# SamsungLabs/fcaf3d

Hardware: AMD Instinct MI355X
Metric: scenes/sec fwd+bwd, ScanNet 100k-pt 2cm voxels, 1/2/4/8 MI355X (higher is better)
Workload: dtype f32

## Files before the change

fcaf3d_amd/_lib.py:

```python
import ctypes
import os
import re
import threading
import time

import torch

_HERE = os.path.dirname(os.path.abspath(__file__))
LIB_PATH = os.environ.get('FC_LIB') or os.path.join(_HERE, 'libfcaf3d_hip.so')
HEADER = os.path.join(os.path.dirname(_HERE), 'include', 'fcaf3d_hip.h')

_SCALARS = {'int': ctypes.c_int, 'int64_t': ctypes.c_int64, 'float': ctypes.c_float,
            'hipStream_t': ctypes.c_void_p}


def parse_header(path=HEADER):
    txt = open(path).read()
    txt = re.sub(r'/\*.*?\*/', '', txt, flags=re.S)
    protos = {}
    for m in re.finditer(r'\b(int64_t|int)\s+(fc_\w+)\s*\(([^)]*)\)\s*;', txt):
        ret, name, args = m.group(1), m.group(2), m.group(3)
        argl = []
        for a in args.split(','):
            a = ' '.join(a.split())
# ... 15 lines not shown
    txt = re.sub(r'//[^\n]*', '', open(path).read())
    known, blocks = {}, []
    for m in re.finditer(r'\benum\s*\{([^}]*)\}', txt):
        block, nxt = {}, 0
        for item in filter(None, (s.strip() for s in m.group(1).split(','))):
            name, _, expr = (s.strip() for s in item.partition('='))
            if expr:
                nxt = sum(known[t] if t in known else int(t, 0) for t in (s.strip() for s in expr.split('+')))
            assert re.fullmatch(r'[A-Z]\w*', name) and name not in known, item
            block[name] = known[name] = nxt
            nxt += 1
        blocks.append(block)
    return blocks


ABI_VERSION = 14
_lib = None
_protos = None


def lib():
    global _lib, _protos
    if _lib is None:
        if not os.path.exists(LIB_PATH):
            raise RuntimeError(
                f'{LIB_PATH} is missing: build it with `python -m fcaf3d_amd.build` '
                '(hipcc --offload-arch=gfx950).  There is no CPU fallback.')
        l = ctypes.CDLL(LIB_PATH)
        _protos = parse_header()
        for name, (ret, args) in _protos.items():
            fn = getattr(l, name)
# ... 119 lines not shown
```

fcaf3d_amd/csrc/exec.hip:

```cpp
#include "fc_common.h"
#include "../../include/fcaf3d_hip.h"
#include "exec_ops.h"
#include <vector>

namespace {

constexpr int MAX_EVENTS = 64;

constexpr int MAX_DEVICES = 16;
hipEvent_t g_events_dev[MAX_DEVICES][MAX_EVENTS];
bool g_events_ready[MAX_DEVICES] = {};
thread_local hipEvent_t* g_events = nullptr;

int ensure_events() {
  int dev = 0;
  FC_HIP(hipGetDevice(&dev));
  if (dev < 0 || dev >= MAX_DEVICES) return FC_EINVAL;
  if (!g_events_ready[dev]) {
    for (int i = 0; i < MAX_EVENTS; ++i) FC_HIP(hipEventCreateWithFlags(&g_events_dev[dev][i], hipEventDisableTiming));
    g_events_ready[dev] = true;
  }
  g_events = g_events_dev[dev];
  return 0;
}
// ... 382 lines not shown
    }
    case OP_AMAX: {
      if (c.dry) return 0;
      return fc_amax(P<const float>(c, op[AMAX_X]), c.dims[op[AMAX_N]] * op[AMAX_C], P<unsigned>(c, op[AMAX_SLOT]), st);
    }
    case OP_CLEAR: {
      if (c.dry) return 0;
      FC_HIP(hipMemsetAsync(P<void>(c, op[CLEAR_DST]), 0, (size_t)op[CLEAR_BYTES], st));
      return 0;
    }
    case OP_NORM_POOL_FWD: {
      const int64_t* m = c.maps + op[NORM_POOL_FWD_MAP] * MAPW;
      if (c.dry) return 0;
      if ((int)m[MAP_K] != 8) return FC_EINVAL;
      if (op[NORM_POOL_FWD_AMAX_OUT_P1] > 0) fc_amax_out_hint(P1<unsigned>(c, op[NORM_POOL_FWD_AMAX_OUT_P1]));
      return fc_norm_act_maxpool8_fwd(P<const float>(c, op[NORM_POOL_FWD_X]), P<const int>(c, op[NORM_POOL_FWD_SEG]),
                                      op[NORM_POOL_FWD_SEG] >= 0 ? 4 : 0, (int)op[NORM_POOL_FWD_C], P<const float>(c, op[NORM_POOL_FWD_MEAN]),
                                      P<const float>(c, op[NORM_POOL_FWD_VAR]), (float)as_double(op[NORM_POOL_FWD_EPS]),
                                      P<const float>(c, op[NORM_POOL_FWD_GAMMA]), P<const float>(c, op[NORM_POOL_FWD_BETA]),
                                      (int)op[NORM_POOL_FWD_ACT], reinterpret_cast<const int*>(m[MAP_NBR]), m[MAP_N_OUT],
                                      P<float>(c, op[NORM_POOL_FWD_OUT]), P<int>(c, op[NORM_POOL_FWD_ARG]), P<float>(c, op[NORM_POOL_FWD_Y]),
                                      P<int>(c, op[NORM_POOL_FWD_PARENT]), st);
    }
    case OP_POOL_NORM_BWD: {
      const int64_t n = c.dims[op[POOL_NORM_BWD_N]];
      const int C = (int)op[POOL_NORM_BWD_C], nseg = (int)c.dims[op[POOL_NORM_BWD_NSEG]];
      if (!want_ws(c, s, fc_maxpool8_norm_act_bwd_ws_bytes(n, C, nseg))) return 0;
      return fc_maxpool8_norm_act_bwd(P<const float>(c, op[POOL_NORM_BWD_X]), P<const float>(c, op[POOL_NORM_BWD_G_POOL]),
                                      P<const int>(c, op[POOL_NORM_BWD_ARG]), P<const int>(c, op[POOL_NORM_BWD_PARENT]),
                                      P<const int>(c, op[POOL_NORM_BWD_SEG]), op[POOL_NORM_BWD_SEG] >= 0 ? 4 : 0, n, C, nseg,
                                      P<const float>(c, op[POOL_NORM_BWD_MEAN]), P<const float>(c, op[POOL_NORM_BWD_VAR]),
                                      P<const float>(c, op[POOL_NORM_BWD_CNT]), (float)as_double(op[POOL_NORM_BWD_EPS]),
                                      P<const float>(c, op[POOL_NORM_BWD_GAMMA]), P<const float>(c, op[POOL_NORM_BWD_BETA]),
                                      (int)op[POOL_NORM_BWD_ACT], P<float>(c, op[POOL_NORM_BWD_GX]), P<float>(c, op[POOL_NORM_BWD_SUMS]),
                                      c.ws[s], c.ws_bytes[s], st);
    }
    case OP_INV_ROWS: {
      if (c.dry) return 0;
      return fc_inverse_rows(P<const int>(c, op[INV_ROWS_ROWS]), c.dims[op[INV_ROWS_N]], c.dims[op[INV_ROWS_N_INV]], P<int>(c, op[INV_ROWS_INV]), st);
    }
    case OP_COPY: {
      if (c.dry) return 0;
// ... 72 lines not shown
```

fcaf3d_amd/csrc/exec_ops.h:

```cpp
#ifndef FCAF3D_EXEC_OPS_H
#define FCAF3D_EXEC_OPS_H

enum {
  OPW = 24,
  MAPW = 20,
  NSTREAM = 3
};
enum { ROW_OP, ROW_STREAM };

enum {
  OP_STEM_FWD = 1, OP_COL_STATS, OP_NORM_FWD, OP_MAXPOOL_FWD, OP_CONV, OP_BN_FWD, OP_UNION_FWD, OP_HEAD_FWD, OP_RECORD, OP_WAIT,
  OP_HEAD_BWD, OP_WGRAD, OP_BN_BWD, OP_NORM_BWD, OP_MAXPOOL_BWD, OP_STEM_WGRAD, OP_GATHER, OP_ADD, OP_SMALL_GRADS,
  OP_PERMUTE_GENT, OP_HEAD_WFIN, OP_COPY, OP_COL_SUM, OP_ROW_SUM, OP_AMAX, OP_CLEAR, OP_NORM_POOL_FWD, OP_POOL_NORM_BWD, OP_INV_ROWS
};

enum {
  STEM_FWD_X = 2,
  STEM_FWD_W,
  STEM_FWD_MAP,
  STEM_FWD_OUT,
  STEM_FWD_COL,
  STEM_FWD_END
};
enum {
// ... 206 lines not shown
  NORM_POOL_FWD_X = 2,
  NORM_POOL_FWD_SEG,
  NORM_POOL_FWD_C,
  NORM_POOL_FWD_MEAN,
  NORM_POOL_FWD_VAR,
  NORM_POOL_FWD_EPS,
  NORM_POOL_FWD_GAMMA,
  NORM_POOL_FWD_BETA,
  NORM_POOL_FWD_ACT,
  NORM_POOL_FWD_MAP,
  NORM_POOL_FWD_OUT,
  NORM_POOL_FWD_ARG,
  NORM_POOL_FWD_Y,
  NORM_POOL_FWD_AMAX_OUT_P1,
  NORM_POOL_FWD_PARENT,
  NORM_POOL_FWD_END
};
enum {
  POOL_NORM_BWD_X = 2,
  POOL_NORM_BWD_G_POOL,
  POOL_NORM_BWD_ARG,
  POOL_NORM_BWD_PARENT,
  POOL_NORM_BWD_SEG,
  POOL_NORM_BWD_N,
  POOL_NORM_BWD_C,
  POOL_NORM_BWD_NSEG,
  POOL_NORM_BWD_MEAN,
  POOL_NORM_BWD_VAR,
  POOL_NORM_BWD_CNT,
  POOL_NORM_BWD_EPS,
  POOL_NORM_BWD_GAMMA,
  POOL_NORM_BWD_BETA,
  POOL_NORM_BWD_ACT,
  POOL_NORM_BWD_GX,
  POOL_NORM_BWD_SUMS,
  POOL_NORM_BWD_END
};
enum {
  INV_ROWS_ROWS = 2,
  INV_ROWS_N,
  INV_ROWS_N_INV,
  INV_ROWS_INV,
  INV_ROWS_END
};

static_assert(STEM_FWD_END <= OPW && COL_STATS_END <= OPW && CONV_END <= OPW && BN_FWD_END <= OPW && HEAD_FWD_END <= OPW, "operator row");
static_assert(RECORD_END <= OPW && WAIT_END <= OPW && HEAD_BWD_END <= OPW && WGRAD_END <= OPW && BN_BWD_END <= OPW, "operator row");
static_assert(STEM_WGRAD_END <= OPW && GATHER_END <= OPW && ADD_END <= OPW && SMALL_GRADS_END <= OPW && PERMUTE_GENT_END <= OPW, "operator row");
static_assert(HEAD_WFIN_END <= OPW && COPY_END <= OPW && COL_SUM_END <= OPW && ROW_SUM_END <= OPW && AMAX_END <= OPW, "operator row");
static_assert(CLEAR_END <= OPW && NORM_POOL_FWD_END <= OPW && POOL_NORM_BWD_END <= OPW && INV_ROWS_END <= OPW, "operator row");
// ... 33 lines not shown
```

fcaf3d_amd/csrc/norm.hip:

```cpp
#include "fc_common.h"
#include "../../include/fcaf3d_hip.h"
#include "norm_route.h"

__device__ static inline int seg_of(const int* seg, int seg_stride, int64_t row) {
  return seg ? seg[row * seg_stride] : 0;
}

__device__ static inline void seg_range(const int* seg, int seg_stride, int64_t r0, int64_t r1, int* lo, int* hi,
                                        int* sh ) {
  if (!seg) { *lo = 0; *hi = 0; return; }
  if (threadIdx.x == 0) { sh[0] = 0x7fffffff; sh[1] = -1; }
  __syncthreads();
  int l = 0x7fffffff, h = -1;
  for (int64_t r = r0 + threadIdx.x; r < r1; r += blockDim.x) {
    int s = seg[r * seg_stride];
    l = s < l ? s : l;
    h = s > h ? s : h;
  }
  if (h >= 0) { atomicMin(&sh[0], l); atomicMax(&sh[1], h); }
  __syncthreads();
  *lo = sh[0]; *hi = sh[1];
  __syncthreads();
}

// ... 210 lines not shown
  if (residual) {
    float4 rs = *reinterpret_cast<const float4*>(residual + r * C + c);
    o.x += rs.x; o.y += rs.y; o.z += rs.z; o.w += rs.w;
  }
  o.x = act_fwd(o.x, act); o.y = act_fwd(o.y, act); o.z = act_fwd(o.z, act); o.w = act_fwd(o.w, act);
  if (q >= 0) {
    const float4 f = *reinterpret_cast<const float4*>(add_src + (int64_t)q * C + c);
    o.x += f.x; o.y += f.y; o.z += f.z; o.w += f.w;
  }
  *reinterpret_cast<float4*>(y + r * C + c) = o;
  amax_fold(am, o.x); amax_fold(am, o.y); amax_fold(am, o.z); amax_fold(am, o.w);
  }
  if (amax_out) amax_commit(am, amax_out);
}

template <bool POOL>
__global__ void k_norm_bwd_partial(const float* __restrict__ x, const float* __restrict__ y, const float* __restrict__ gy,
                                   const float* __restrict__ gy2, const int* __restrict__ pool_parent,
                                   const int* __restrict__ pool_arg, const int* __restrict__ seg, int seg_stride, int64_t n, int C, int nseg,
                                   const float* __restrict__ mean, const float* __restrict__ var, float eps, int act,
                                   const float* __restrict__ gamma, const float* __restrict__ beta,
                                   int64_t rpb, float* __restrict__ part) {
  extern __shared__ float sm[];
  __shared__ int srange[2];
  const int c4n = C / 4;
  const int cl = threadIdx.x % c4n, rl = threadIdx.x / c4n;
  const int nrl = blockDim.x / c4n;
  const int64_t r0 = (int64_t)blockIdx.x * rpb;
  int64_t r1 = r0 + rpb;
  if (r1 > n) r1 = n;
  int s_lo, s_hi;
// ... 9 lines not shown
      float4 is = make_float4(1.f / sqrtf(va.x + eps), 1.f / sqrtf(va.y + eps), 1.f / sqrtf(va.z + eps),
                              1.f / sqrtf(va.w + eps));
      const float4 gm = gamma ? *reinterpret_cast<const float4*>(gamma + cl * 4) : make_float4(1.f, 1.f, 1.f, 1.f);
      const float4 bt = beta ? *reinterpret_cast<const float4*>(beta + cl * 4) : make_float4(0.f, 0.f, 0.f, 0.f);
      const bool from_y = act && y;
      for (int64_t rb = r0 + rl; rb < r1; rb += 4 * nrl) {
        float4 xv[4], gv[4], yv[4], g2[4];
        bool ok[4];
#pragma unroll
        for (int u = 0; u < 4; ++u) {
          const int64_t r = rb + (int64_t)u * nrl;
          ok[u] = r < r1;
          const int64_t rc = ok[u] ? r : r0;
          if (chk) ok[u] = ok[u] && seg[rc * seg_stride] == s;
          xv[u] = *reinterpret_cast<const float4*>(x + rc * C + cl * 4);
          if (POOL) {
            const int64_t o = pool_parent[rc];
            const int4 a = *reinterpret_cast<const int4*>(pool_arg + o * C + cl * 4);
            gv[u] = *reinterpret_cast<const float4*>(gy + o * C + cl * 4);
            gv[u].x = a.x == rc ? gv[u].x : 0.f; gv[u].y = a.y == rc ? gv[u].y : 0.f;
            gv[u].z = a.z == rc ? gv[u].z : 0.f; gv[u].w = a.w == rc ? gv[u].w : 0.f;
          } else {
            gv[u] = *reinterpret_cast<const float4*>(gy + rc * C + cl * 4);
          }
          if (gy2) g2[u] = *reinterpret_cast<const float4*>(gy2 + rc * C + cl * 4);
          if (from_y) yv[u] = *reinterpret_cast<const float4*>(y + rc * C + cl * 4);
        }
#pragma unroll
        for (int u = 0; u < 4; ++u) {
          if (!ok[u]) continue;
          float4 g = gv[u];
// ... 24 lines not shown
    if (rl == 0) {
      float4 t1 = make_float4(0.f, 0.f, 0.f, 0.f), t2 = t1;
      for (int j = 0; j < nrl; ++j) {
        float4 u = *reinterpret_cast<const float4*>(&sm[(j * 2 + 0) * C + cl * 4]);
        float4 w = *reinterpret_cast<const float4*>(&sm[(j * 2 + 1) * C + cl * 4]);
        t1.x += u.x; t1.y += u.y; t1.z += u.z; t1.w += u.w;
        t2.x += w.x; t2.y += w.y; t2.z += w.z; t2.w += w.w;
      }
      float* dst = part + (((int64_t)blockIdx.x * nseg + s) * 2) * C;
      *reinterpret_cast<float4*>(dst + cl * 4) = t1;
      *reinterpret_cast<float4*>(dst + C + cl * 4) = t2;
    }
  }
}

template <bool POOL>
__global__ void k_norm_bwd_apply(const float* __restrict__ x, const float* __restrict__ y, const float* __restrict__ gy,
                                 const float* __restrict__ gy2, const int* __restrict__ pool_parent,
                                 const int* __restrict__ pool_arg, const int* __restrict__ seg, int seg_stride, int64_t n, int C,
                                 const float* __restrict__ mean, const float* __restrict__ var, float eps,
                                 const float* __restrict__ gamma, const float* __restrict__ beta,
                                 const float* __restrict__ sums ,
                                 const float* __restrict__ cnt, int act, float* __restrict__ gx, float* __restrict__ gres,
                                 unsigned* __restrict__ amax_out) {
  int64_t t = (int64_t)blockIdx.x * blockDim.x + threadIdx.x;
  const int c4n = C / 4;
  unsigned am = 0u;
  if (t < n * c4n) {
  int64_t r = t / c4n;
  int c = (int)(t % c4n) * 4;
  int s = seg_of(seg, seg_stride, r);
  float inv_n = 1.f / cnt[s];
  float xv[4], gv[4], muv[4], vav[4], gam[4], bet[4] = {0.f, 0.f, 0.f, 0.f}, s1[4], s2[4], yv[4], o[4], gr[4];
  *reinterpret_cast<float4*>(xv) = *reinterpret_cast<const float4*>(x + r * C + c);
  if (POOL) {
    const int64_t o = pool_parent[r];
    const int4 a = *reinterpret_cast<const int4*>(pool_arg + o * C + c);
    *reinterpret_cast<float4*>(gv) = *reinterpret_cast<const float4*>(gy + o * C + c);
    gv[0] = a.x == r ? gv[0] : 0.f; gv[1] = a.y == r ? gv[1] : 0.f; gv[2] = a.z == r ? gv[2] : 0.f; gv[3] = a.w == r ? gv[3] : 0.f;
  } else {
    *reinterpret_cast<float4*>(gv) = *reinterpret_cast<const float4*>(gy + r * C + c);
  }
  if (gy2) {
    const float4 t2 = *reinterpret_cast<const float4*>(gy2 + r * C + c);
    gv[0] += t2.x; gv[1] += t2.y; gv[2] += t2.z; gv[3] += t2.w;
  }
  *reinterpret_cast<float4*>(muv) = *reinterpret_cast<const float4*>(mean + (int64_t)s * C + c);
  *reinterpret_cast<float4*>(vav) = *reinterpret_cast<const float4*>(var + (int64_t)s * C + c);
  *reinterpret_cast<float4*>(s1) = *reinterpret_cast<const float4*>(sums + ((int64_t)s * 2) * C + c);
  *reinterpret_cast<float4*>(s2) = *reinterpret_cast<const float4*>(sums + ((int64_t)s * 2 + 1) * C + c);
// ... 69 lines not shown
  *reinterpret_cast<float4*>(out + o * C + c) = ob;
  *reinterpret_cast<int4*>(argrow + o * C + c) = make_int4(arg[0], arg[1], arg[2], arg[3]);
  amax_fold(am, ob.x); amax_fold(am, ob.y); amax_fold(am, ob.z); amax_fold(am, ob.w);
  }
  if (amax_out) amax_commit(am, amax_out);
}

__global__ void k_maxpool_bwd(const float* __restrict__ gout, const int* __restrict__ argrow, int64_t n_out, int C,
                              float* __restrict__ gin) {
  int64_t t = (int64_t)blockIdx.x * blockDim.x + threadIdx.x;
  if (t >= n_out * C) return;
  int i = argrow[t];
  if (i >= 0) gin[(int64_t)i * C + (t % C)] = gout[t];
}

__global__ void k_norm_act_maxpool8_fwd(const float* __restrict__ x, const int* __restrict__ seg, int seg_stride, int C,
                                        const float* __restrict__ mean, const float* __restrict__ var, float eps,
                                        const float* __restrict__ gamma, const float* __restrict__ beta, int act,
                                        const int* __restrict__ nbr, int64_t n_out, float* __restrict__ out, int* __restrict__ argrow,
                                        float* __restrict__ y, int* __restrict__ parent, unsigned* __restrict__ amax_out) {
  const int c4n = C / 4;
  int64_t t = (int64_t)blockIdx.x * blockDim.x + threadIdx.x;
  unsigned am = 0u;
  if (t < n_out * c4n) {
  const int64_t o = t / c4n;
  const int c = (int)(t % c4n) * 4;
  int idx[8];
#pragma unroll
  for (int k = 0; k < 8; ++k) idx[k] = nbr[(int64_t)k * n_out + o];
  if (parent) {
    int mine = -1;
#pragma unroll
    for (int k = 0; k < 8; ++k) mine = (c == 4 * k) ? idx[k] : mine;
    if (mine >= 0) parent[mine] = (int)o;
  }
  float4 v[8];
  int first = -1;
#pragma unroll
  for (int k = 0; k < 8; ++k) {
    const int i = idx[k] < 0 ? 0 : idx[k];
    if (first < 0 && idx[k] >= 0) first = idx[k];
    v[k] = *reinterpret_cast<const float4*>(x + (int64_t)i * C + c);
  }
  float best[4] = {-INFINITY, -INFINITY, -INFINITY, -INFINITY};
  int arg[4] = {-1, -1, -1, -1};
  if (first >= 0) {
    const int s = seg_of(seg, seg_stride, first);
    float mu[4], va[4], is[4], g[4] = {1.f, 1.f, 1.f, 1.f}, b[4] = {0.f, 0.f, 0.f, 0.f};
    *reinterpret_cast<float4*>(mu) = *reinterpret_cast<const float4*>(mean + (int64_t)s * C + c);
// ... 4 lines not shown
    for (int j = 0; j < 4; ++j) is[j] = 1.f / sqrtf(va[j] + eps);
#pragma unroll
    for (int k = 0; k < 8; ++k) {
      if (idx[k] < 0) continue;
      float e[4] = {v[k].x, v[k].y, v[k].z, v[k].w};
#pragma unroll
      for (int j = 0; j < 4; ++j) {
        e[j] = act_fwd(bn_pre(e[j], mu[j], is[j], g[j], b[j]), act);
        if (arg[j] < 0 || e[j] > best[j]) { best[j] = e[j]; arg[j] = idx[k]; }
      }
      if (y) *reinterpret_cast<float4*>(y + (int64_t)idx[k] * C + c) = make_float4(e[0], e[1], e[2], e[3]);
    }
  }
  float4 ob = make_float4(arg[0] < 0 ? 0.f : best[0], arg[1] < 0 ? 0.f : best[1], arg[2] < 0 ? 0.f : best[2], arg[3] < 0 ? 0.f : best[3]);
  *reinterpret_cast<float4*>(out + o * C + c) = ob;
  *reinterpret_cast<int4*>(argrow + o * C + c) = make_int4(arg[0], arg[1], arg[2], arg[3]);
  amax_fold(am, ob.x); amax_fold(am, ob.y); amax_fold(am, ob.z); amax_fold(am, ob.w);
  }
  if (amax_out) amax_commit(am, amax_out);
}

__global__ void k_inverse_rows(const int* __restrict__ rows, int64_t n, int64_t n_inv, int* __restrict__ inv) {
  const int64_t i = (int64_t)blockIdx.x * blockDim.x + threadIdx.x;
  if (i >= n) return;
  const int r = rows[i];
  if (r >= 0 && r < n_inv) inv[r] = (int)i;
}

__global__ void k_gather_rows(const float* __restrict__ src, const int* __restrict__ idx, int64_t n, int C,
                              float* __restrict__ dst) {
  int64_t t = (int64_t)blockIdx.x * blockDim.x + threadIdx.x;
// ... 456 lines not shown
    FC_CHECK_LAUNCH();
  }
  if (!apply) return FC_OK;
  if (r.apply == FC_NAPPLY_BN1)
    k_bn1_apply<<<FC_GRID(r.ap, stream)>>>(x, n, C, r.rpb, part, (int)r.np, eps, gamma, beta, residual, act, momentum, y, mean, var, cnt, rmean, rvar, nbt, add_inv, add_src);
  else if (r.apply == FC_NAPPLY_BN2)
    k_bn2_apply<<<FC_GRID(r.ap, stream)>>>(x, n, C, r.rpb, table, (int)r.np, groups, eps, gamma, beta, residual, act, momentum, y, mean, var, cnt, rmean, rvar, nbt, r.cg,
                                   add_inv, add_src, amax);
  else
    k_norm_act_fwd<<<FC_GRID(r.ap, stream)>>>(x, nullptr, 0, n, C, mean, var, eps, gamma, beta, residual, act, add_inv, add_src, y, amax);
  FC_CHECK_LAUNCH();
  if (r.amax == FC_NAMAX_PASS && amax) return fc_amax(y, n * (int64_t)C, amax, stream);
  return FC_OK;
}

template <bool POOL>
static int norm_bwd(int form, const float* x, const float* y, const float* gy, const float* gy2, const int* parent, const int* argrow, const int* seg,
                    int seg_stride, int64_t n, int C, int nseg, const float* mean, const float* var, const float* cnt, float eps, const float* gamma,
                    const float* beta, int act, float* gx, float* gres, float* sums, const float* table, int64_t nb_part, int64_t small_elems, void* ws,
                    int64_t ws_bytes, hipStream_t stream, unsigned* amax, bool late_hint = false) {
  if (act < 0 || act > 2) return FC_EINVAL;
  const NormRoute r = norm_bwd_route(n, C, nseg, table != nullptr, nb_part, small_elems, form);
  if (int rc = route_check(r, ws_bytes)) return rc;
  if (late_hint) amax = take_amax_out();
  if (r.apply == FC_NBAPPLY_NONE) {
    FC_HIP(hipMemsetAsync(sums, 0, sizeof(float) * nseg * 2 * C, stream));
    return FC_OK;
  }
  if (r.sums == FC_NRED_PARTIAL) {
    k_norm_bwd_partial<POOL><<<FC_GRID(r.red, stream)>>>(x, y, gy, gy2, parent, argrow, seg, seg_stride, n, C, nseg, mean, var, eps, act, gamma, beta, r.red_rpb, (float*)ws);
    FC_CHECK_LAUNCH();
// ... 93 lines not shown
  return bn_fwd(x, n, C, 0.f, nullptr, nullptr, nullptr, 0, momentum, nullptr, mean, var, cnt, running_mean, running_var, num_batches_tracked, nullptr, 0, 1,
                -1, nullptr, nullptr, ws, ws_bytes, stream, nullptr, false);
}

int fc_bn_act_train_fwd(const float* x, int64_t n, int C, float eps, const float* gamma, const float* beta,
                        const float* residual, int act, float momentum, float* y, float* mean, float* var, float* cnt,
                        float* running_mean, float* running_var, long long* num_batches_tracked, void* ws,
                        int64_t ws_bytes, hipStream_t stream) {
  return bn_fwd(x, n, C, eps, gamma, beta, residual, act, momentum, y, mean, var, cnt, running_mean, running_var, num_batches_tracked, nullptr, 0, 1,
                INT64_MAX, nullptr, nullptr, ws, ws_bytes, stream, nullptr);
}

int fc_bn_act_train_bwd(const float* x, const float* y, const float* gy, int64_t n, int C, const float* mean,
                        const float* var, float eps, const float* gamma, const float* beta, int act, float* gx, float* gres,
                        float* sums, void* ws, int64_t ws_bytes, hipStream_t stream) {
  return norm_bwd<false>(FC_NFORM_SMALL, x, y, gy, nullptr, nullptr, nullptr, nullptr, 0, n, C, 1, mean, var, nullptr, eps, gamma, beta, act, gx, gres, sums,
                         nullptr, 0, 0, ws, ws_bytes, stream, nullptr, true);
}

int fc_norm_act_add_fwd(const float* x, const int* seg, int seg_stride, int64_t n, int C, const float* mean, const float* var,
                        float eps, const float* gamma, const float* beta, const float* residual, int act, const int* add_inv,
                        const float* add_src, float* y, hipStream_t stream) {
  unsigned* ao = take_amax_out();
  if (n < 0 || C < 4 || C % 4 || act < 0 || act > 2 || (add_inv == nullptr) != (add_src == nullptr)) return FC_EINVAL;
  if (n == 0) return FC_OK;
  k_norm_act_fwd<<<FC_GRID(rows_launch(n, C), stream)>>>(x, seg, seg_stride, n, C, mean, var, eps, gamma, beta, residual, act, add_inv, add_src, y, ao);
  FC_CHECK_LAUNCH();
  return FC_OK;
}

int fc_norm_act_fwd(const float* x, const int* seg, int seg_stride, int64_t n, int C, const float* mean, const float* var,
                    float eps, const float* gamma, const float* beta, const float* residual, int act, float* y,
                    hipStream_t stream) {
  unsigned* ao = take_amax_out();
  if (n < 0 || C < 4 || C % 4 || act < 0 || act > 2) return FC_EINVAL;
  if (n == 0) return FC_OK;
  k_norm_act_fwd<<<FC_GRID(rows_launch(n, C), stream)>>>(x, seg, seg_stride, n, C, mean, var, eps, gamma, beta, residual, act, nullptr, nullptr, y, ao);
  FC_CHECK_LAUNCH();
  return FC_OK;
}

int fc_norm_act_bwd(const float* x, const float* y, const float* gy, const int* seg, int seg_stride, int64_t n, int C,
                    int nseg, const float* mean, const float* var, const float* cnt, float eps, const float* gamma,
                    const float* beta, int act, float* gx, float* gres, float* sums, void* ws, int64_t ws_bytes,
                    hipStream_t stream) {
  unsigned* ao = take_amax_out();
  return norm_bwd<false>(FC_NFORM_SEG, x, y, gy, nullptr, nullptr, nullptr, seg, seg_stride, n, C, nseg, mean, var, cnt, eps, gamma, beta, act, gx, gres, sums,
                         nullptr, 0, 0, ws, ws_bytes, stream, ao);
}

int fc_bn_train_add_fwd(const float* x, int64_t n, int C, float eps, const float* gamma, const float* beta, const float* residual,
                        int act, float momentum, float* y, float* mean, float* var, float* cnt, float* running_mean,
                        float* running_var, long long* num_batches_tracked, const float* part, int64_t nb_part, int groups,
                        int64_t small_elems, const int* add_inv, const float* add_src, void* ws, int64_t ws_bytes,
                        hipStream_t stream) {
  unsigned* ao = take_amax_out();
  return bn_fwd(x, n, C, eps, gamma, beta, residual, act, momentum, y, mean, var, cnt, running_mean, running_var, num_batches_tracked, part, nb_part, groups,
                small_elems, add_inv, add_src, ws, ws_bytes, stream, ao);
}

int fc_bn_train_fwd(const float* x, int64_t n, int C, float eps, const float* gamma, const float* beta, const float* residual,
                    int act, float momentum, float* y, float* mean, float* var, float* cnt, float* running_mean,
                    float* running_var, long long* num_batches_tracked, const float* part, int64_t nb_part, int groups,
                    int64_t small_elems, void* ws, int64_t ws_bytes, hipStream_t stream) {
  unsigned* ao = take_amax_out();
  return bn_fwd(x, n, C, eps, gamma, beta, residual, act, momentum, y, mean, var, cnt, running_mean, running_var, num_batches_tracked, part, nb_part, groups,
                small_elems, nullptr, nullptr, ws, ws_bytes, stream, ao);
}

int fc_bn_train_bwd(const float* x, const float* y, const float* gy, const float* gy2, int64_t n, int C, const float* mean,
                    const float* var, const float* cnt, float eps, const float* gamma, const float* beta, int act, float* gx,
                    float* gres, float* sums, const float* part, int64_t nb_part, int64_t small_elems, void* ws, int64_t ws_bytes,
                    hipStream_t stream) {
  unsigned* ao = take_amax_out();
  return norm_bwd<false>(FC_NFORM_TRAIN, x, y, gy, gy2, nullptr, nullptr, nullptr, 0, n, C, 1, mean, var, cnt, eps, gamma, beta, act, gx, gres, sums, part, nb_part,
                         small_elems, ws, ws_bytes, stream, ao);
}

int fc_amax_out_hint(unsigned* amax_word) {
  t_fc_amax_out = amax_word;
  return FC_OK;
}

int fc_maxpool_fwd(const float* in, const int* nbr, int64_t n_out, int K, int C, float* out, int* argrow,
                   hipStream_t stream) {
  unsigned* ao = take_amax_out();
  if (n_out < 0 || K < 1 || C < 1) return FC_EINVAL;
  if (n_out == 0) return FC_OK;
  if (K == 8 && C % 4 == 0) k_maxpool8_fwd<<<(unsigned)fc_cdiv(n_out * (C / 4), 256), 256, 0, stream>>>(in, nbr, n_out, C, out, argrow, ao);
  else k_maxpool_fwd<<<(unsigned)fc_cdiv(n_out * C, 256), 256, 0, stream>>>(in, nbr, n_out, K, C, out, argrow);
// ... 20 lines not shown

int fc_scatter_rows_add(const float* src, const int* idx, int64_t n, int C, float* dst, hipStream_t stream) {
  if (n < 0 || C < 1) return FC_EINVAL;
  if (n == 0) return FC_OK;
  k_scatter_rows_add<<<(unsigned)fc_cdiv(n * C, 256), 256, 0, stream>>>(src, idx, n, C, dst);
  FC_CHECK_LAUNCH();
  return FC_OK;
}

int fc_norm_act_maxpool8_fwd(const float* x, const int* seg, int seg_stride, int C, const float* mean, const float* var, float eps,
                             const float* gamma, const float* beta, int act, const int* nbr, int64_t n_out, float* out,
                             int* argrow, float* y, int* parent, hipStream_t stream) {
  unsigned* ao = take_amax_out();
  if (n_out < 0 || C < 4 || C % 4 || act < 0 || act > 2) return FC_EINVAL;
  if (n_out == 0) return FC_OK;
  k_norm_act_maxpool8_fwd<<<(unsigned)fc_cdiv(n_out * (C / 4), 256), 256, 0, stream>>>(x, seg, seg_stride, C, mean, var, eps, gamma, beta,
                                                                                      act, nbr, n_out, out, argrow, y, parent, ao);
  FC_CHECK_LAUNCH();
  return FC_OK;
}

int fc_maxpool8_norm_act_bwd(const float* x, const float* gout, const int* argrow, const int* parent, const int* seg, int seg_stride,
                             int64_t n_in, int C, int nseg, const float* mean, const float* var, const float* cnt, float eps,
                             const float* gamma, const float* beta, int act, float* gx, float* sums, void* ws, int64_t ws_bytes,
                             hipStream_t stream) {
  if (!parent || !argrow) return FC_EINVAL;
  return norm_bwd<true>(FC_NFORM_SEG, x, nullptr, gout, nullptr, parent, argrow, seg, seg_stride, n_in, C, nseg, mean, var, cnt, eps, gamma, beta, act, gx, nullptr,
                        sums, nullptr, 0, 0, ws, ws_bytes, stream, nullptr);
}

int fc_inverse_rows(const int* rows, int64_t n, int64_t n_inv, int* inv, hipStream_t stream) {
  if (n < 0 || n_inv < 0) return FC_EINVAL;
  if (n_inv > 0) FC_HIP(hipMemsetAsync(inv, 0xff, sizeof(int) * n_inv, stream));
  if (n == 0) return FC_OK;
  k_inverse_rows<<<(unsigned)fc_cdiv(n, 256), 256, 0, stream>>>(rows, n, n_inv, inv);
  FC_CHECK_LAUNCH();
  return FC_OK;
}

}
```

fcaf3d_amd/executor.py:

```python
import os
import struct

import numpy as np
import torch

from . import _lib as L
from . import functional as Fn
from . import nn as MEnn

ENABLED = os.environ.get('FC_EXEC', '1') != '0'
PROBE = None
TRUSTED = None
KEEP_STATE = False


def _layouts():
    names, fields = {}, {}
    for block in L.parse_enums():
        names.update(block)
        *members, end = block
        op = names.get('OP_' + end[:-len('_END')]) if end.endswith('_END') else None
        if op is not None:
            fields[op] = {n[len(end) - 3:].lower().removesuffix('_p1'): (block[n], n.endswith('_P1')) for n in members}
    return {k: v for k, v in names.items() if k.startswith('OP_') or k in ('OPW', 'MAPW', 'ROW_OP', 'ROW_STREAM')}, fields
# ... 664 lines not shown
                G.arrive(res, gres, rows, C, stream)
        self.tape.append(bwd)
        return y

    def stem(self, stem, inorm):
        p, F, tr, relu = self.p, self.F, self.tr, Fn.ACT['relu']
        x0, seg1 = p.DY('x0'), p.DY('seg1')
        t_stem = p.T('n1', 64)
        col = p.T('n1', 84) if tr else -1
        p.emit(F, OP_STEM_FWD, S_MAIN, x=x0, w=p.S(stem.kernel), map=p.M('stem'), out=t_stem, col=col)
        mean_in, var_in, cnt_in = p.T('B', 64), p.T('B', 64), p.T('B', 1)
        p.emit(F, OP_COL_STATS, S_MAIN, x=t_stem, seg=seg1, n=p.D('n1'), c=64, nseg=p.D('B'), mean=mean_in, var=var_in, cnt=cnt_in)
        t_in = p.T('n1', 64) if p.keep_state else -1
        if p.keep_state:
            p.relu_outs.append((t_in, 'n1', 64))
        t_pool, arg = p.T('n2', 64), p.T('n2', 64)
        p.pool_arg = (arg, 'n2', 64)
        ap = self.folded(t_pool)
        pool_parent = p.T('n1', 1) if tr else -1
        p.emit(F, OP_NORM_POOL_FWD, S_MAIN, x=t_stem, seg=seg1, c=64, mean=mean_in, var=var_in, eps=_f(inorm.eps), gamma=p.S(inorm.weight),
               beta=p.S(inorm.bias), act=relu, map=p.M('pool'), out=t_pool, arg=arg, y=t_in, amax_out=ap, parent=pool_parent)
        if tr:
            p.in_sums = p.T('B', 2 * 64, 'b')

            def bwd():
                p.small.append((None, 'B', 64, inorm.weight, inorm.bias))
                g_pool = self.grads.take(t_pool, 'n2', 64)
                g_stem = p.T('n1', 64, 'b')
                p.emit(self.Bk, OP_POOL_NORM_BWD, S_MAIN, x=t_stem, g_pool=g_pool, arg=arg, parent=pool_parent, seg=seg1, n=p.D('n1'), c=64,
                       nseg=p.D('B'), mean=mean_in, var=var_in, cnt=cnt_in, eps=_f(inorm.eps), gamma=p.S(inorm.weight),
                       beta=p.S(inorm.bias), act=relu, gx=g_stem, sums=p.in_sums)
                self.wgrad(S_MAIN, OP_STEM_WGRAD, col=col, gout=g_stem, map=p.M('stem'), gw=p.G(stem.kernel))
                self.wrote(stem.kernel)
            self.tape.append(bwd)
        return t_pool, 'n2', 64

    def level(self, li, layer, x):
        relu, none, N = Fn.ACT['relu'], Fn.ACT['none'], _Names
        (cur, cur_rows, _), rows = x, N.rows(li)
        if self.tr:
            self.tape.append(lambda: self.flush_small(S_MAIN))
        for j, blk in enumerate(layer):
            if j == 0:
                assert blk.downsample is not None and blk.conv1.stride == 2
                t_ds = self.conv(cur, cur_rows, rows, blk.downsample[0], N.ds(li))
                res = self.bn(t_ds, blk.downsample[1], none, rows)
# ... 181 lines not shown
```

include/fcaf3d_hip.h:

```cpp
#ifndef FCAF3D_HIP_H
#define FCAF3D_HIP_H
#include <stdint.h>

#ifndef __HIP_PLATFORM_AMD__
typedef struct ihipStream_t* hipStream_t;
#endif

#ifdef __cplusplus
extern "C" {
#endif

#define FC_ABI_VERSION 14
#ifndef FC_AMAX_SLOT_BYTES
#define FC_AMAX_SLOT_BYTES 2048
#endif
int fc_abi_version(void);


int fc_voxelize(const float* points, int64_t n, int pt_stride, int batch_idx, float voxel_size, float feat_div,
                int nfeat, int* coords, float* feats, hipStream_t stream);

int fc_augment_voxelize(const float* points, int64_t n_src, int pt_stride, const int* sample_idx, int64_t n_out,
                        const float* xform_host, int batch_idx, float voxel_size, float feat_div, int nfeat, int* coords,
                        float* feats, float* points_out, hipStream_t stream);

#define FC_BATCH_DESC_WORDS 18
int fc_batch_augment_voxelize(const float* arena, int64_t arena_rows, int pt_stride, const int64_t* desc, int B, int64_t total_out,
// ... 187 lines not shown
int fc_bn_train_bwd_route(int64_t n, int C, int nseg, int has_part, int64_t nb_part, int64_t small_elems, int form, int* out);

int fc_maxpool_fwd(const float* in, const int* nbr, int64_t n_out, int K, int C, float* out, int* argrow,
                   hipStream_t stream);
int fc_maxpool_bwd(const float* gout, const int* argrow, int64_t n_out, int C, float* gin, hipStream_t stream);

int fc_norm_act_maxpool8_fwd(const float* x, const int* seg, int seg_stride, int C, const float* mean, const float* var, float eps,
                             const float* gamma, const float* beta, int act, const int* nbr, int64_t n_out, float* out,
                             int* argrow, float* y, int* parent, hipStream_t stream);
int64_t fc_maxpool8_norm_act_bwd_ws_bytes(int64_t n_in, int C, int nseg);
int fc_maxpool8_norm_act_bwd(const float* x, const float* gout, const int* argrow, const int* parent, const int* seg, int seg_stride,
                             int64_t n_in, int C, int nseg, const float* mean, const float* var, const float* cnt, float eps,
                             const float* gamma, const float* beta, int act, float* gx, float* sums, void* ws, int64_t ws_bytes,
                             hipStream_t stream);

int fc_inverse_rows(const int* rows, int64_t n, int64_t n_inv, int* inv, hipStream_t stream);
int fc_norm_act_add_fwd(const float* x, const int* seg, int seg_stride, int64_t n, int C, const float* mean, const float* var,
                        float eps, const float* gamma, const float* beta, const float* residual, int act, const int* add_inv,
                        const float* add_src, float* y, hipStream_t stream);
int fc_bn_train_add_fwd(const float* x, int64_t n, int C, float eps, const float* gamma, const float* beta, const float* residual,
                        int act, float momentum, float* y, float* mean, float* var, float* cnt, float* running_mean,
                        float* running_var, long long* num_batches_tracked, const float* part, int64_t nb_part, int groups,
                        int64_t small_elems, const int* add_inv, const float* add_src, void* ws, int64_t ws_bytes,
                        hipStream_t stream);

int fc_gather_rows(const float* src, const int* idx, int64_t n, int C, float* dst, hipStream_t stream);
int fc_scatter_rows_add(const float* src, const int* idx, int64_t n, int C, float* dst, hipStream_t stream);


int fc_focal_loss_fwd(const float* logits, const long long* labels, const float* row_weight, int64_t n, int C, float gamma,
// ... 101 lines not shown
```

Before: 517.8.

## Replace stem maxpool argrow tensor with compact per-slot win bitmask

During training the stem norm+ReLU+maxpool8 kernel now writes a 4-bit-per-channel bitmask of which of the 8 children won, instead of a full int32 argrow tensor per output channel. The backward norm kernels decode this mask using a parent index that packs output row and child slot. This cuts the argrow write and read traffic from 256 bytes to 64 bytes per pooled row. In exchange the mask path only supports C=64, adds shuffle work in the forward kernel, and still keeps argrow when state must be retained.

```diff
diff --git a/fcaf3d_amd/_lib.py b/fcaf3d_amd/_lib.py
--- a/fcaf3d_amd/_lib.py
+++ b/fcaf3d_amd/_lib.py
@@ -53,7 +53,7 @@
     return blocks
 
 
-ABI_VERSION = 14
+ABI_VERSION = 15
 _lib = None
 _protos = None
 
diff --git a/fcaf3d_amd/csrc/exec.hip b/fcaf3d_amd/csrc/exec.hip
--- a/fcaf3d_amd/csrc/exec.hip
+++ b/fcaf3d_amd/csrc/exec.hip
@@ -420,6 +420,14 @@
       if (c.dry) return 0;
       if ((int)m[MAP_K] != 8) return FC_EINVAL;
       if (op[NORM_POOL_FWD_AMAX_OUT_P1] > 0) fc_amax_out_hint(P1<unsigned>(c, op[NORM_POOL_FWD_AMAX_OUT_P1]));
+      if (op[NORM_POOL_FWD_MASK_P1] > 0)
+        return fc_norm_act_maxpool8_mask_fwd(P<const float>(c, op[NORM_POOL_FWD_X]), P<const int>(c, op[NORM_POOL_FWD_SEG]),
+                                             op[NORM_POOL_FWD_SEG] >= 0 ? 4 : 0, (int)op[NORM_POOL_FWD_C], P<const float>(c, op[NORM_POOL_FWD_MEAN]),
+                                             P<const float>(c, op[NORM_POOL_FWD_VAR]), (float)as_double(op[NORM_POOL_FWD_EPS]),
+                                             P<const float>(c, op[NORM_POOL_FWD_GAMMA]), P<const float>(c, op[NORM_POOL_FWD_BETA]),
+                                             (int)op[NORM_POOL_FWD_ACT], reinterpret_cast<const int*>(m[MAP_NBR]), m[MAP_N_OUT],
+                                             P<float>(c, op[NORM_POOL_FWD_OUT]), P<int>(c, op[NORM_POOL_FWD_ARG]), P<float>(c, op[NORM_POOL_FWD_Y]),
+                                             P<int>(c, op[NORM_POOL_FWD_PARENT]), P1<void>(c, op[NORM_POOL_FWD_MASK_P1]), st);
       return fc_norm_act_maxpool8_fwd(P<const float>(c, op[NORM_POOL_FWD_X]), P<const int>(c, op[NORM_POOL_FWD_SEG]),
                                       op[NORM_POOL_FWD_SEG] >= 0 ? 4 : 0, (int)op[NORM_POOL_FWD_C], P<const float>(c, op[NORM_POOL_FWD_MEAN]),
                                       P<const float>(c, op[NORM_POOL_FWD_VAR]), (float)as_double(op[NORM_POOL_FWD_EPS]),
@@ -432,6 +440,15 @@
       const int64_t n = c.dims[op[POOL_NORM_BWD_N]];
       const int C = (int)op[POOL_NORM_BWD_C], nseg = (int)c.dims[op[POOL_NORM_BWD_NSEG]];
       if (!want_ws(c, s, fc_maxpool8_norm_act_bwd_ws_bytes(n, C, nseg))) return 0;
+      if (op[POOL_NORM_BWD_MASK_P1] > 0)
+        return fc_maxpool8_mask_norm_act_bwd(P<const float>(c, op[POOL_NORM_BWD_X]), P<const float>(c, op[POOL_NORM_BWD_G_POOL]),
+                                             P1<const void>(c, op[POOL_NORM_BWD_MASK_P1]), P<const int>(c, op[POOL_NORM_BWD_PARENT]),
+                                             P<const int>(c, op[POOL_NORM_BWD_SEG]), op[POOL_NORM_BWD_SEG] >= 0 ? 4 : 0, n, C, nseg,
+                                             P<const float>(c, op[POOL_NORM_BWD_MEAN]), P<const float>(c, op[POOL_NORM_BWD_VAR]),
+                                             P<const float>(c, op[POOL_NORM_BWD_CNT]), (float)as_double(op[POOL_NORM_BWD_EPS]),
+                                             P<const float>(c, op[POOL_NORM_BWD_GAMMA]), P<const float>(c, op[POOL_NORM_BWD_BETA]),
+                                             (int)op[POOL_NORM_BWD_ACT], P<float>(c, op[POOL_NORM_BWD_GX]), P<float>(c, op[POOL_NORM_BWD_SUMS]),
+                                             c.ws[s], c.ws_bytes[s], st);
       return fc_maxpool8_norm_act_bwd(P<const float>(c, op[POOL_NORM_BWD_X]), P<const float>(c, op[POOL_NORM_BWD_G_POOL]),
                                       P<const int>(c, op[POOL_NORM_BWD_ARG]), P<const int>(c, op[POOL_NORM_BWD_PARENT]),
                                       P<const int>(c, op[POOL_NORM_BWD_SEG]), op[POOL_NORM_BWD_SEG] >= 0 ? 4 : 0, n, C, nseg,
diff --git a/fcaf3d_amd/csrc/exec_ops.h b/fcaf3d_amd/csrc/exec_ops.h
--- a/fcaf3d_amd/csrc/exec_ops.h
+++ b/fcaf3d_amd/csrc/exec_ops.h
@@ -244,6 +244,7 @@
   NORM_POOL_FWD_Y,
   NORM_POOL_FWD_AMAX_OUT_P1,
   NORM_POOL_FWD_PARENT,
+  NORM_POOL_FWD_MASK_P1,
   NORM_POOL_FWD_END
 };
 enum {
@@ -264,6 +265,7 @@
   POOL_NORM_BWD_ACT,
   POOL_NORM_BWD_GX,
   POOL_NORM_BWD_SUMS,
+  POOL_NORM_BWD_MASK_P1,
   POOL_NORM_BWD_END
 };
 enum {
diff --git a/fcaf3d_amd/csrc/norm.hip b/fcaf3d_amd/csrc/norm.hip
--- a/fcaf3d_amd/csrc/norm.hip
+++ b/fcaf3d_amd/csrc/norm.hip
@@ -248,7 +248,8 @@
   if (amax_out) amax_commit(am, amax_out);
 }
 
-template <bool POOL>
+enum { FC_POOL_NONE = 0, FC_POOL_ARG = 1, FC_POOL_MASK = 2 };
+template <int POOL>
 __global__ void k_norm_bwd_partial(const float* __restrict__ x, const float* __restrict__ y, const float* __restrict__ gy,
                                    const float* __restrict__ gy2, const int* __restrict__ pool_parent,
                                    const int* __restrict__ pool_arg, const int* __restrict__ seg, int seg_stride, int64_t n, int C, int nseg,
@@ -288,7 +289,14 @@
           const int64_t rc = ok[u] ? r : r0;
           if (chk) ok[u] = ok[u] && seg[rc * seg_stride] == s;
           xv[u] = *reinterpret_cast<const float4*>(x + rc * C + cl * 4);
-          if (POOL) {
+          if (POOL == FC_POOL_MASK) {
+            const int64_t p8 = pool_parent[rc];
+            const int64_t o = p8 >> 3;
+            const unsigned m = reinterpret_cast<const unsigned*>(pool_arg)[p8 * 2 + (cl >> 3)] >> (4 * (cl & 7));
+            gv[u] = *reinterpret_cast<const float4*>(gy + o * C + cl * 4);
+            gv[u].x = (m & 1u) ? gv[u].x : 0.f; gv[u].y = (m & 2u) ? gv[u].y : 0.f;
+            gv[u].z = (m & 4u) ? gv[u].z : 0.f; gv[u].w = (m & 8u) ? gv[u].w : 0.f;
+          } else if (POOL == FC_POOL_ARG) {
             const int64_t o = pool_parent[rc];
             const int4 a = *reinterpret_cast<const int4*>(pool_arg + o * C + cl * 4);
             gv[u] = *reinterpret_cast<const float4*>(gy + o * C + cl * 4);
@@ -343,7 +351,7 @@
   }
 }
 
-template <bool POOL>
+template <int POOL>
 __global__ void k_norm_bwd_apply(const float* __restrict__ x, const float* __restrict__ y, const float* __restrict__ gy,
                                  const float* __restrict__ gy2, const int* __restrict__ pool_parent,
                                  const int* __restrict__ pool_arg, const int* __restrict__ seg, int seg_stride, int64_t n, int C,
@@ -362,7 +370,13 @@
   float inv_n = 1.f / cnt[s];
   float xv[4], gv[4], muv[4], vav[4], gam[4], bet[4] = {0.f, 0.f, 0.f, 0.f}, s1[4], s2[4], yv[4], o[4], gr[4];
   *reinterpret_cast<float4*>(xv) = *reinterpret_cast<const float4*>(x + r * C + c);
-  if (POOL) {
+  if (POOL == FC_POOL_MASK) {
+    const int64_t p8 = pool_parent[r];
+    const int64_t o = p8 >> 3;
+    const unsigned m = reinterpret_cast<const unsigned*>(pool_arg)[p8 * 2 + (c >> 5)] >> (c & 28);
+    *reinterpret_cast<float4*>(gv) = *reinterpret_cast<const float4*>(gy + o * C + c);
+    gv[0] = (m & 1u) ? gv[0] : 0.f; gv[1] = (m & 2u) ? gv[1] : 0.f; gv[2] = (m & 4u) ? gv[2] : 0.f; gv[3] = (m & 8u) ? gv[3] : 0.f;
+  } else if (POOL == FC_POOL_ARG) {
     const int64_t o = pool_parent[r];
     const int4 a = *reinterpret_cast<const int4*>(pool_arg + o * C + c);
     *reinterpret_cast<float4*>(gv) = *reinterpret_cast<const float4*>(gy + o * C + c);
@@ -462,11 +476,13 @@
   if (i >= 0) gin[(int64_t)i * C + (t % C)] = gout[t];
 }
 
+template <bool MASK>
 __global__ void k_norm_act_maxpool8_fwd(const float* __restrict__ x, const int* __restrict__ seg, int seg_stride, int C,
                                         const float* __restrict__ mean, const float* __restrict__ var, float eps,
                                         const float* __restrict__ gamma, const float* __restrict__ beta, int act,
                                         const int* __restrict__ nbr, int64_t n_out, float* __restrict__ out, int* __restrict__ argrow,
-                                        float* __restrict__ y, int* __restrict__ parent, unsigned* __restrict__ amax_out) {
+                                        float* __restrict__ y, int* __restrict__ parent, unsigned* __restrict__ mask,
+                                        unsigned* __restrict__ amax_out) {
   const int c4n = C / 4;
   int64_t t = (int64_t)blockIdx.x * blockDim.x + threadIdx.x;
   unsigned am = 0u;
@@ -480,7 +496,7 @@
     int mine = -1;
 #pragma unroll
     for (int k = 0; k < 8; ++k) mine = (c == 4 * k) ? idx[k] : mine;
-    if (mine >= 0) parent[mine] = (int)o;
+    if (mine >= 0) parent[mine] = MASK ? (int)(o * 8 + c / 4) : (int)o;
   }
   float4 v[8];
   int first = -1;
@@ -515,7 +531,19 @@
   }
   float4 ob = make_float4(arg[0] < 0 ? 0.f : best[0], arg[1] < 0 ? 0.f : best[1], arg[2] < 0 ? 0.f : best[2], arg[3] < 0 ? 0.f : best[3]);
   *reinterpret_cast<float4*>(out + o * C + c) = ob;
-  *reinterpret_cast<int4*>(argrow + o * C + c) = make_int4(arg[0], arg[1], arg[2], arg[3]);
+  if (!MASK || argrow) *reinterpret_cast<int4*>(argrow + o * C + c) = make_int4(arg[0], arg[1], arg[2], arg[3]);
+  if (MASK) {
+    unsigned won = 0u;
+#pragma unroll
+    for (int k = 0; k < 8; ++k)
+#pragma unroll
+      for (int j = 0; j < 4; ++j) won |= (idx[k] >= 0 && arg[j] == idx[k]) ? 1u << (4 * k + j) : 0u;
+    const int cl = c >> 2, k = cl & 7;
+    unsigned w = 0u;
+#pragma unroll
+    for (int i = 0; i < 8; ++i) w |= ((__shfl(won, (cl & 8) + i, 16) >> (4 * k)) & 15u) << (4 * i);
+    mask[(o * 8 + k) * 2 + (cl >> 3)] = w;
+  }
   amax_fold(am, ob.x); amax_fold(am, ob.y); amax_fold(am, ob.z); amax_fold(am, ob.w);
   }
   if (amax_out) amax_commit(am, amax_out);
@@ -1002,7 +1030,7 @@
   return FC_OK;
 }
 
-template <bool POOL>
+template <int POOL>
 static int norm_bwd(int form, const float* x, const float* y, const float* gy, const float* gy2, const int* parent, const int* argrow, const int* seg,
                     int seg_stride, int64_t n, int C, int nseg, const float* mean, const float* var, const float* cnt, float eps, const float* gamma,
                     const float* beta, int act, float* gx, float* gres, float* sums, const float* table, int64_t nb_part, int64_t small_elems, void* ws,
@@ -1126,7 +1154,7 @@
 int fc_bn_act_train_bwd(const float* x, const float* y, const float* gy, int64_t n, int C, const float* mean,
                         const float* var, float eps, const float* gamma, const float* beta, int act, float* gx, float* gres,
                         float* sums, void* ws, int64_t ws_bytes, hipStream_t stream) {
-  return norm_bwd<false>(FC_NFORM_SMALL, x, y, gy, nullptr, nullptr, nullptr, nullptr, 0, n, C, 1, mean, var, nullptr, eps, gamma, beta, act, gx, gres, sums,
+  return norm_bwd<FC_POOL_NONE>(FC_NFORM_SMALL, x, y, gy, nullptr, nullptr, nullptr, nullptr, 0, n, C, 1, mean, var, nullptr, eps, gamma, beta, act, gx, gres, sums,
                          nullptr, 0, 0, ws, ws_bytes, stream, nullptr, true);
 }
 
@@ -1157,7 +1185,7 @@
                     const float* beta, int act, float* gx, float* gres, float* sums, void* ws, int64_t ws_bytes,
                     hipStream_t stream) {
   unsigned* ao = take_amax_out();
-  return norm_bwd<false>(FC_NFORM_SEG, x, y, gy, nullptr, nullptr, nullptr, seg, seg_stride, n, C, nseg, mean, var, cnt, eps, gamma, beta, act, gx, gres, sums,
+  return norm_bwd<FC_POOL_NONE>(FC_NFORM_SEG, x, y, gy, nullptr, nullptr, nullptr, seg, seg_stride, n, C, nseg, mean, var, cnt, eps, gamma, beta, act, gx, gres, sums,
                          nullptr, 0, 0, ws, ws_bytes, stream, ao);
 }
 
@@ -1185,7 +1213,7 @@
                     float* gres, float* sums, const float* part, int64_t nb_part, int64_t small_elems, void* ws, int64_t ws_bytes,
                     hipStream_t stream) {
   unsigned* ao = take_amax_out();
-  return norm_bwd<false>(FC_NFORM_TRAIN, x, y, gy, gy2, nullptr, nullptr, nullptr, 0, n, C, 1, mean, var, cnt, eps, gamma, beta, act, gx, gres, sums, part, nb_part,
+  return norm_bwd<FC_POOL_NONE>(FC_NFORM_TRAIN, x, y, gy, gy2, nullptr, nullptr, nullptr, 0, n, C, 1, mean, var, cnt, eps, gamma, beta, act, gx, gres, sums, part, nb_part,
                          small_elems, ws, ws_bytes, stream, ao);
 }
 
@@ -1236,8 +1264,9 @@
   unsigned* ao = take_amax_out();
   if (n_out < 0 || C < 4 || C % 4 || act < 0 || act > 2) return FC_EINVAL;
   if (n_out == 0) return FC_OK;
-  k_norm_act_maxpool8_fwd<<<(unsigned)fc_cdiv(n_out * (C / 4), 256), 256, 0, stream>>>(x, seg, seg_stride, C, mean, var, eps, gamma, beta,
-                                                                                      act, nbr, n_out, out, argrow, y, parent, ao);
+  k_norm_act_maxpool8_fwd<false><<<(unsigned)fc_cdiv(n_out * (C / 4), 256), 256, 0, stream>>>(x, seg, seg_stride, C, mean, var, eps, gamma,
+                                                                                             beta, act, nbr, n_out, out, argrow, y, parent,
+                                                                                             nullptr, ao);
   FC_CHECK_LAUNCH();
   return FC_OK;
 }
@@ -1247,8 +1276,32 @@
                              const float* gamma, const float* beta, int act, float* gx, float* sums, void* ws, int64_t ws_bytes,
                              hipStream_t stream) {
   if (!parent || !argrow) return FC_EINVAL;
-  return norm_bwd<true>(FC_NFORM_SEG, x, nullptr, gout, nullptr, parent, argrow, seg, seg_stride, n_in, C, nseg, mean, var, cnt, eps, gamma, beta, act, gx, nullptr,
+  return norm_bwd<FC_POOL_ARG>(FC_NFORM_SEG, x, nullptr, gout, nullptr, parent, argrow, seg, seg_stride, n_in, C, nseg, mean, var, cnt, eps, gamma, beta, act, gx, nullptr,
                         sums, nullptr, 0, 0, ws, ws_bytes, stream, nullptr);
+}
+
+int64_t fc_maxpool8_mask_bytes(int64_t n_out) { return (n_out < 0 || n_out > FC_POOL_MASK_MAX_ROWS) ? -1 : n_out * 64; }
+
+int fc_norm_act_maxpool8_mask_fwd(const float* x, const int* seg, int seg_stride, int C, const float* mean, const float* var, float eps,
+                                  const float* gamma, const float* beta, int act, const int* nbr, int64_t n_out, float* out,
+                                  int* argrow, float* y, int* parent, void* mask, hipStream_t stream) {
+  unsigned* ao = take_amax_out();
+  if (n_out < 0 || n_out > FC_POOL_MASK_MAX_ROWS || C != 64 || act < 0 || act > 2 || !parent || !mask) return FC_EINVAL;
+  if (n_out == 0) return FC_OK;
+  k_norm_act_maxpool8_fwd<true><<<(unsigned)fc_cdiv(n_out * 16, 256), 256, 0, stream>>>(x, seg, seg_stride, C, mean, var, eps, gamma, beta,
+                                                                                       act, nbr, n_out, out, argrow, y, parent,
+                                                                                       (unsigned*)mask, ao);
+  FC_CHECK_LAUNCH();
+  return FC_OK;
+}
+
+int fc_maxpool8_mask_norm_act_bwd(const float* x, const float* gout, const void* mask, const int* parent, const int* seg, int seg_stride,
+                                  int64_t n_in, int C, int nseg, const float* mean, const float* var, const float* cnt, float eps,
+                                  const float* gamma, const float* beta, int act, float* gx, float* sums, void* ws, int64_t ws_bytes,
+                                  hipStream_t stream) {
+  if (!parent || !mask || C != 64) return FC_EINVAL;
+  return norm_bwd<FC_POOL_MASK>(FC_NFORM_SEG, x, nullptr, gout, nullptr, parent, (const int*)mask, seg, seg_stride, n_in, C, nseg, mean, var, cnt, eps, gamma,
+                                beta, act, gx, nullptr, sums, nullptr, 0, 0, ws, ws_bytes, stream, nullptr);
 }
 
 int fc_inverse_rows(const int* rows, int64_t n, int64_t n_inv, int* inv, hipStream_t stream) {
diff --git a/fcaf3d_amd/executor.py b/fcaf3d_amd/executor.py
--- a/fcaf3d_amd/executor.py
+++ b/fcaf3d_amd/executor.py
@@ -702,12 +702,15 @@
         t_in = p.T('n1', 64) if p.keep_state else -1
         if p.keep_state:
             p.relu_outs.append((t_in, 'n1', 64))
-        t_pool, arg = p.T('n2', 64), p.T('n2', 64)
-        p.pool_arg = (arg, 'n2', 64)
+        t_pool = p.T('n2', 64)
+        arg = p.T('n2', 64) if p.keep_state or not tr else -1
+        mask = p.T('n2', 16) if tr else -1
+        if arg >= 0:
+            p.pool_arg = (arg, 'n2', 64)
         ap = self.folded(t_pool)
         pool_parent = p.T('n1', 1) if tr else -1
         p.emit(F, OP_NORM_POOL_FWD, S_MAIN, x=t_stem, seg=seg1, c=64, mean=mean_in, var=var_in, eps=_f(inorm.eps), gamma=p.S(inorm.weight),
-               beta=p.S(inorm.bias), act=relu, map=p.M('pool'), out=t_pool, arg=arg, y=t_in, amax_out=ap, parent=pool_parent)
+               beta=p.S(inorm.bias), act=relu, map=p.M('pool'), out=t_pool, arg=arg, y=t_in, amax_out=ap, parent=pool_parent, mask=mask)
         if tr:
             p.in_sums = p.T('B', 2 * 64, 'b')
 
@@ -715,9 +718,9 @@
                 p.small.append((None, 'B', 64, inorm.weight, inorm.bias))
                 g_pool = self.grads.take(t_pool, 'n2', 64)
                 g_stem = p.T('n1', 64, 'b')
-                p.emit(self.Bk, OP_POOL_NORM_BWD, S_MAIN, x=t_stem, g_pool=g_pool, arg=arg, parent=pool_parent, seg=seg1, n=p.D('n1'), c=64,
+                p.emit(self.Bk, OP_POOL_NORM_BWD, S_MAIN, x=t_stem, g_pool=g_pool, arg=-1, parent=pool_parent, seg=seg1, n=p.D('n1'), c=64,
                        nseg=p.D('B'), mean=mean_in, var=var_in, cnt=cnt_in, eps=_f(inorm.eps), gamma=p.S(inorm.weight),
-                       beta=p.S(inorm.bias), act=relu, gx=g_stem, sums=p.in_sums)
+                       beta=p.S(inorm.bias), act=relu, gx=g_stem, sums=p.in_sums, mask=mask)
                 self.wgrad(S_MAIN, OP_STEM_WGRAD, col=col, gout=g_stem, map=p.M('stem'), gw=p.G(stem.kernel))
                 self.wrote(stem.kernel)
             self.tape.append(bwd)
diff --git a/include/fcaf3d_hip.h b/include/fcaf3d_hip.h
--- a/include/fcaf3d_hip.h
+++ b/include/fcaf3d_hip.h
@@ -10,7 +10,7 @@
 extern "C" {
 #endif
 
-#define FC_ABI_VERSION 14
+#define FC_ABI_VERSION 15
 #ifndef FC_AMAX_SLOT_BYTES
 #define FC_AMAX_SLOT_BYTES 2048
 #endif
@@ -228,6 +228,16 @@
                              const float* gamma, const float* beta, int act, float* gx, float* sums, void* ws, int64_t ws_bytes,
                              hipStream_t stream);
 
+#define FC_POOL_MASK_MAX_ROWS ((int64_t)1 << 28)
+int64_t fc_maxpool8_mask_bytes(int64_t n_out);
+int fc_norm_act_maxpool8_mask_fwd(const float* x, const int* seg, int seg_stride, int C, const float* mean, const float* var, float eps,
+                                  const float* gamma, const float* beta, int act, const int* nbr, int64_t n_out, float* out,
+                                  int* argrow, float* y, int* parent, void* mask, hipStream_t stream);
+int fc_maxpool8_mask_norm_act_bwd(const float* x, const float* gout, const void* mask, const int* parent, const int* seg, int seg_stride,
+                                  int64_t n_in, int C, int nseg, const float* mean, const float* var, const float* cnt, float eps,
+                                  const float* gamma, const float* beta, int act, float* gx, float* sums, void* ws, int64_t ws_bytes,
+                                  hipStream_t stream);
+
 int fc_inverse_rows(const int* rows, int64_t n, int64_t n_inv, int* inv, hipStream_t stream);
 int fc_norm_act_add_fwd(const float* x, const int* seg, int seg_stride, int64_t n, int C, const float* mean, const float* var,
                         float eps, const float* gamma, const float* beta, const float* residual, int act, const int* add_inv,
```

New measurement: 519.2, median of 6. Within noise of the previous version (+0.3%).
